# GDMCF/GDMCF

Hardware: AMD Instinct MI355X
Metric: training users/sec (higher is better)
Workload: dtype f32; 1 GPU; yelp-shape synthetic rows, batch=400/GPU, dims=[1000], T=5, noise_scale=0.01, linear-var, mean_type=x0, reweight, AdamW lr=1e-5 (BASELINE configs[1]); n_items=34395, global_batch=400, parallelism=dp1, batch_rows=device CSR rows (CsrBatch)

## Files before the change

gdmcf_amd/csrc/common.h:

```cpp
#pragma once
#include <hip/hip_runtime.h>
#include <stdint.h>
#include <stdio.h>

#include "../../include/gdmcf_hip.h"

typedef float f32x4 __attribute__((ext_vector_type(4)));
typedef f32x4 f32x4_u4 __attribute__((aligned(4)));

void gdmcf_set_error(const char* fmt, ...);

#define GD_CHECK_SHAPE(cond, msg)            \
    do {                                     \
        if (!(cond)) {                       \
            gdmcf_set_error("%s", msg);      \
            return GDMCF_E_SHAPE;            \
        }                                    \
    } while (0)

#define GD_CHECK_ARG(cond, msg)              \
    do {                                     \
        if (!(cond)) {                       \
            gdmcf_set_error("%s", msg);      \
            return GDMCF_E_ARG;              \
// ... 40 lines not shown
    return c;
}

struct GdShadow {
    void* p16;
    int64_t ld16;
    int64_t rows, cols;
};
bool gd_shadow_lookup(const void* f32, GdShadow* out);
int gd_cast_bf16(const float* src, int64_t ld, void* dst, int64_t ld16, int64_t rows, int64_t cols, hipStream_t s);

__device__ __forceinline__ unsigned short gd_bf16_bits(float x) {
    __bf16 h = (__bf16)x;
    return __builtin_bit_cast(unsigned short, h);
}

enum { GD_LAY_KC = 0, GD_LAY_MC = 1 };
enum { GD_EPI_SLAB = 0, GD_EPI_BIAS_ACT = 1, GD_EPI_LOSS = 2, GD_EPI_POST = 3, GD_EPI_STORE = 4, GD_EPI_ADAMW = 5 };

struct GdAdamHyper {
    float decay;
    float one_m_b1;
    float beta2;
    float one_m_b2;
    float bc2_sqrt;
    float eps;
    float neg_step;
    float grad_scale;
    float inv_bc2_sqrt;
    float pad_[3];
// ... 84 lines not shown
```

gdmcf_amd/csrc/linear.hip:

```cpp
#include <stdlib.h>

#include "common.h"

int gd_splitk_reduce(const float* slabs, int64_t slab_stride, int splits, int64_t ld_slab, int M, int N, int mode,
                     const float* bias, const float* rowscale, const float* aact, int64_t ldact, int act, float* out,
                     int64_t ldo, hipStream_t s);
int gd_colsum(const float* dZ, int64_t ld, const float* rs, int M, int N, float* db, hipStream_t s);
int gd_rowpart_reduce(const float* rowpart, int ld, int M, int nt, float* rowsum, hipStream_t s);

namespace {

static const int TARGET_WGS = getenv("GDMCF_TARGET_WGS") ? atoi(getenv("GDMCF_TARGET_WGS")) : 760;

thread_local int t_gemm_prec = GDMCF_GEMM_F32;

int pick_class(int M, int N, bool fused, int prec) {
    if (prec == GDMCF_GEMM_BF16 && M > 128) {
        const long pad = (long)gd_cdiv(M, 208) * 208;
        const long tiles = (pad / 208) * gd_cdiv(N, 256);
        const long rounds = (tiles + 255) / 256;
        if (pad * 10 <= (long)M * 11 && pad / 208 <= 2 && (!fused || tiles * 100 >= rounds * 256 * 85)) return 3;
    }
    if (prec == GDMCF_GEMM_F32X3 && M > 128 && N >= 128) {
        const long pad = (long)gd_cdiv(M, 208) * 208;
// ... 61 lines not shown
    g.bf16 = t_gemm_prec;
    g.A = e.dZ; g.lda = e.lddz; g.B = e.A; g.ldb = e.lda; g.M = N; g.N = K; g.K = M; g.splits = 1;
    g.m_fastest = gd_cdiv(N, gd_gemm_tile_m(cls)) <= gd_cdiv(K, gd_gemm_tile_n(cls));
    g.C = e.W; g.ldc = e.ldw; g.aux = e.exp_avg; g.aux2 = e.exp_avg_sq; g.prof_tag = 5;
    g.adam = gd_adam_hyper(e.lr, e.beta1, e.beta2, e.eps, e.weight_decay, e.step, e.grad_scale);
    g.adam_dev = t_gd_step_state ? &t_gd_step_state->hyper : nullptr;
    attach_result_shadow(g);
    attach_shadows(g, GD_LAY_MC, GD_LAY_MC);
    g.out2 = bias_col_request(e.a_scale_col, e.lda, e.rowscale, K, e.db);
    return GDMCF_OK;
}

int dw_adamw_finish(const GdDwAdamw& e, bool asked, const GdGemm& g, hipStream_t s) {
    if (asked && g.out2 == nullptr) return GDMCF_OK;
    if (e.db) return gd_colsum(e.dZ, e.lddz, e.rowscale, e.M, e.N, e.db, s);
    return GDMCF_OK;
}

}

extern "C" {

int gdmcf_gemm_precision(int mode) {
    const int prev = t_gemm_prec;
    if (mode == GDMCF_GEMM_F32 || mode == GDMCF_GEMM_BF16 || mode == GDMCF_GEMM_F32X3) t_gemm_prec = mode;
    return prev;
}

size_t gdmcf_linear_ws_bytes(int M, int N, int K) {
    if (M <= 0 || N <= 0 || K <= 0) return 0;
// ... 136 lines not shown
    GdGemm g = {};
    g.bf16 = t_gemm_prec;
    g.A = A; g.lda = lda; g.B = W; g.ldb = ldw; g.M = M; g.N = N; g.K = K; g.splits = 1;
    g.m_fastest = gd_cdiv(M, gd_gemm_tile_m(cls)) <= gd_cdiv(N, gd_gemm_tile_n(cls));
    g.bias = bias; g.aux = x_t; g.ldaux = ldxt; g.aux2 = z; g.ldaux2 = ldz;
    g.r0 = c1; g.r1 = c2; g.r2 = r1; g.r3 = r2; g.r4 = sigma;
    g.out2 = pred_out; g.ldout2 = ldp; g.C = x_next; g.ldc = ldxn; g.prof_tag = 3;
    attach_result_shadow(g);
    attach_shadows(g, GD_LAY_KC, GD_LAY_KC);
    return gd_gemm_launch(GD_LAY_KC, GD_LAY_KC, GD_EPI_POST, cls, g, s);
}

int gdmcf_linear_bwd_input_f32(const float* dZ, int64_t lddz, const float* W, int64_t ldw, const float* rowscale,
                               const float* Aact, int64_t ldact, int act, int M, int N, int K, float* dA,
                               int64_t ldda, void* ws, size_t ws_bytes, void* stream) {
    GD_CHECK_SHAPE(M > 0 && N > 0 && K > 0 && lddz >= N && ldw >= K && ldda >= K, "linear_bwd_input: bad shape");
    GD_CHECK_ARG(act == 0 || (act == 1 && Aact && ldact >= K), "linear_bwd_input: activation output missing");
    hipStream_t s = (hipStream_t)stream;
    const int cls = pick_class(M, K, false, t_gemm_prec);
    const int splits = pick_splits(M, K, N, cls, t_gemm_prec);
    const int64_t lds_ = round4(K);
    const size_t need = (size_t)splits * M * lds_ * sizeof(float);
    if (ws == nullptr || ws_bytes < need) {
        gdmcf_set_error("linear_bwd_input: workspace %zu < %zu bytes", ws_bytes, need);
        return GDMCF_E_WORKSPACE;
    }
    GdGemm g = {};
    g.bf16 = t_gemm_prec;
    g.A = dZ; g.lda = lddz; g.B = W; g.ldb = ldw; g.M = M; g.N = K; g.K = N;
    g.m_fastest = gd_cdiv(M, gd_gemm_tile_m(cls)) <= gd_cdiv(K, gd_gemm_tile_n(cls));
    g.splits = splits; g.C = (float*)ws; g.ldc = lds_; g.slab_stride = (int64_t)M * lds_; g.prof_tag = 4;
    g.ws_cap = ws_bytes;
    attach_shadows(g, GD_LAY_KC, GD_LAY_MC);
    int rc = gd_gemm_launch(GD_LAY_KC, GD_LAY_MC, GD_EPI_SLAB, cls, g, s);
    if (rc) return rc;
    const int real_splits = gd_cdiv(N, g.kchunk);
    return gd_splitk_reduce((const float*)ws, g.slab_stride, real_splits, lds_, M, K, 1, nullptr, rowscale, Aact,
                            ldact, act, dA, ldda, s);
}

int gdmcf_linear_bwd_weight_f32(const float* dZ, int64_t lddz, const float* A, int64_t lda, const float* rowscale,
                                int a_scale_col, int M, int N, int K, float* dW, int64_t lddw, float* db, int accumulate,
                                void* stream) {
    GD_CHECK_SHAPE(M > 0 && N > 0 && K > 0 && lddz >= N && lda >= K && lddw >= K, "linear_bwd_weight: bad shape");
    hipStream_t s = (hipStream_t)stream;
    const int cls = pick_class_dw(N, K, t_gemm_prec);
    GdGemm g = {};
    g.bf16 = t_gemm_prec;
    g.A = dZ; g.lda = lddz; g.B = A; g.ldb = lda; g.M = N; g.N = K; g.K = M; g.splits = 1;
    g.m_fastest = gd_cdiv(N, gd_gemm_tile_m(cls)) <= gd_cdiv(K, gd_gemm_tile_n(cls));
    g.C = dW; g.ldc = lddw; g.accumulate = accumulate; g.prof_tag = 5;
    attach_shadows(g, GD_LAY_MC, GD_LAY_MC);
    g.out2 = bias_col_request(a_scale_col, lda, rowscale, K, db);
// ... 60 lines not shown
```

gdmcf_amd/csrc/reduce.hip:

```cpp
#include "common.h"

namespace {

__global__ __launch_bounds__(256) void splitk_reduce_kernel(const float* __restrict__ slabs, int64_t slab_stride,
                                                            int splits, int64_t ld_slab, int M, int N, int mode,
                                                            const float* __restrict__ bias,
                                                            const float* __restrict__ rowscale,
                                                            const float* __restrict__ aact, int64_t ldact, int act,
                                                            float* __restrict__ out, int64_t ldo,
                                                            unsigned short* __restrict__ out16, int64_t ldo16, int vec) {
    const int m = blockIdx.y;
    const int n0 = (blockIdx.x * 256 + threadIdx.x) * 4;
    if (n0 >= N) return;
    float sv[4] = {0.f, 0.f, 0.f, 0.f};
    const float* p = slabs + (int64_t)m * ld_slab + n0;
    if (vec && n0 + 3 < N) {
        for (int k0 = 0; k0 < splits; k0 += 8) {
            f32x4 t[8];
#pragma unroll
            for (int u = 0; u < 8; ++u)
                t[u] = (k0 + u < splits) ? *reinterpret_cast<const f32x4*>(p + (int64_t)(k0 + u) * slab_stride)
                                         : f32x4{0.f, 0.f, 0.f, 0.f};
#pragma unroll
            for (int u = 0; u < 8; ++u)
                if (k0 + u < splits) { sv[0] += t[u].x; sv[1] += t[u].y; sv[2] += t[u].z; sv[3] += t[u].w; }
        }
    } else {
// ... 7 lines not shown
        const int n = n0 + j;
        if (n >= N) break;
        float s = sv[j];
        if (mode == 0) {
            if (bias) s += bias[n];
            if (act == 1) s = tanhf(s);
        } else {
            if (rowscale) s *= rs;
            if (act == 1) {
                const float h = aact[(int64_t)m * ldact + n];
                s *= (1.f - h * h);
            }
        }
        out[(int64_t)m * ldo + n] = s;
        if (out16) out16[(int64_t)m * ldo16 + n] = gd_bf16_bits(s);
    }
}

__global__ __launch_bounds__(256) void rowscale_kernel(const float* __restrict__ A, int64_t lda,
                                                       const float* __restrict__ rs, int M, int K,
                                                       float* __restrict__ out, int64_t ldo,
                                                       unsigned short* __restrict__ out16, int64_t ldo16, int bias_col) {
    const int m = blockIdx.y, k = (blockIdx.x * 256 + threadIdx.x) * 4;
    if (bias_col && blockIdx.x == 0 && threadIdx.x == 0) out[(int64_t)m * ldo + K] = rs[m];
    if (k >= K) return;
    const float r = rs[m];
    const float* a = A + (int64_t)m * lda + k;
    float* o = out + (int64_t)m * ldo + k;
    float v[4];
    if (k + 3 < K) {
        const f32x4 t = *reinterpret_cast<const f32x4_u4*>(a);
        v[0] = t.x * r; v[1] = t.y * r; v[2] = t.z * r; v[3] = t.w * r;
        *reinterpret_cast<f32x4_u4*>(o) = f32x4{v[0], v[1], v[2], v[3]};
    } else {
        for (int j = 0; j < 4; ++j)
            if (k + j < K) o[j] = v[j] = a[j] * r;
    }
    if (out16)
        for (int j = 0; j < 4; ++j)
            if (k + j < K) out16[(int64_t)m * ldo16 + k + j] = gd_bf16_bits(v[j]);
}

__global__ __launch_bounds__(256) void colsum_kernel(const float* __restrict__ dZ, int64_t ld,
                                                     const float* __restrict__ rs, int M, int N,
                                                     float* __restrict__ db) {
    __shared__ float part[4][64];
    const int lane = threadIdx.x & 63, wave = threadIdx.x >> 6;
    const int n = blockIdx.x * 64 + lane;
    const int nc = min(n, N - 1);
    float s = 0.f;
    int m = wave;
    for (; m + 28 < M; m += 32) {
        float v[8];
#pragma unroll
        for (int j = 0; j < 8; ++j) v[j] = dZ[(int64_t)(m + 4 * j) * ld + nc] * (rs ? rs[m + 4 * j] : 1.f);
#pragma unroll
        for (int j = 0; j < 8; ++j) s += v[j];
// ... 58 lines not shown

}

int gd_splitk_reduce(const float* slabs, int64_t slab_stride, int splits, int64_t ld_slab, int M, int N, int mode,
                     const float* bias, const float* rowscale, const float* aact, int64_t ldact, int act, float* out,
                     int64_t ldo, hipStream_t s) {
    GdShadow sh;
    const bool has16 = gd_shadow_lookup(out, &sh) && sh.rows == M && sh.cols == N;
    const int vec = (ld_slab % 4 == 0) && (slab_stride % 4 == 0) && gd_aligned16(slabs);
    hipLaunchKernelGGL(splitk_reduce_kernel, dim3(gd_cdiv(N, 1024), M), dim3(256), 0, s, slabs, slab_stride,
                       splits, ld_slab, M, N, mode, bias, rowscale, aact, ldact, act, out, ldo,
                       has16 ? (unsigned short*)sh.p16 : nullptr, has16 ? sh.ld16 : 0, vec);
    return gd_launch_status("splitk_reduce");
}

int gd_colsum(const float* dZ, int64_t ld, const float* rs, int M, int N, float* db, hipStream_t s) {
    hipLaunchKernelGGL(colsum_kernel, dim3(gd_cdiv(N, 64)), dim3(256), 0, s, dZ, ld, rs, M, N, db);
    return gd_launch_status("colsum");
}

int gd_rowpart_reduce(const float* rowpart, int ld, int M, int nt, float* rowsum, hipStream_t s) {
    hipLaunchKernelGGL(rowpart_reduce_kernel, dim3(gd_cdiv(M, 4)), dim3(256), 0, s, rowpart, ld, M, nt, rowsum);
    return gd_launch_status("rowpart_reduce");
}

int gd_cast_bf16(const float* src, int64_t ld, void* dst, int64_t ld16, int64_t rows, int64_t cols, hipStream_t s) {
    const int64_t total = rows * ((cols + 7) / 8);
    const int64_t blocks = (total + 255) / 256;
    hipLaunchKernelGGL(cast_bf16_kernel, dim3((unsigned)(blocks < 16384 ? blocks : 16384)), dim3(256), 0, s, src, ld,
                       (unsigned short*)dst, ld16, rows, cols);
// ... 3 lines not shown
```

gdmcf_amd/csrc/rows.hip:

```cpp
#include "common.h"

namespace {

__device__ __forceinline__ float block_sum_256(float v, float* red) {
#pragma unroll
    for (int o = 32; o > 0; o >>= 1) v += __shfl_down(v, o, 64);
    __syncthreads();
    if ((threadIdx.x & 63) == 0) red[threadIdx.x >> 6] = v;
    __syncthreads();
    return red[0] + red[1] + red[2] + red[3];
}

__global__ __launch_bounds__(256) void row_norms_kernel(const float* __restrict__ X, int64_t ld, int cols,
                                                       float* __restrict__ norm, float* __restrict__ inv_norm) {
    __shared__ float red[4];
    const float* x = X + (int64_t)blockIdx.x * ld;
    float ss = 0.f;
    const int c4 = cols & ~3;
    for (int c = threadIdx.x * 4; c < c4; c += 1024) {
        const f32x4 t = *reinterpret_cast<const f32x4_u4*>(x + c);
        ss += t.x * t.x + t.y * t.y + t.z * t.z + t.w * t.w;
    }
    if (threadIdx.x < cols - c4) ss += x[c4 + threadIdx.x] * x[c4 + threadIdx.x];
    const float n = sqrtf(block_sum_256(ss, red));
// ... 155 lines not shown
}

__global__ __launch_bounds__(256) void emb_gather_w_kernel(const float* __restrict__ W1, int64_t ldw, int I, int E, int N,
                                                           float* __restrict__ W1e) {
    const int idx = blockIdx.x * 256 + threadIdx.x;
    if (idx < N * E) W1e[idx] = W1[(int64_t)(idx / E) * ldw + I + (idx % E)];
}

__global__ __launch_bounds__(256) void emb_bwd_demb_kernel(const float* __restrict__ dZ1, int64_t lddz,
                                                           const float* __restrict__ W1e, int E, int N,
                                                           float* __restrict__ demb) {
    const int m = blockIdx.x;
    const int lane = threadIdx.x & 63, wave = threadIdx.x >> 6;
    for (int e = wave; e < E; e += 4) {
        float s = 0.f;
        for (int n = lane; n < N; n += 64) s += dZ1[(int64_t)m * lddz + n] * W1e[(int64_t)n * E + e];
        for (int o = 32; o > 0; o >>= 1) s += __shfl_xor(s, o);
        if (lane == 0) demb[(int64_t)m * E + e] = s;
    }
}

__global__ __launch_bounds__(64) void emb_bwd_w_kernel(const float* __restrict__ demb, const float* __restrict__ temb,
                                                       int M, int E, float* __restrict__ dWe,
                                                       float* __restrict__ dbe) {
    const int idx = blockIdx.x, lane = threadIdx.x;
    float s = 0.f;
    if (idx < E * E) {
        const int e = idx / E, f = idx % E;
        for (int m = lane; m < M; m += 64) s += demb[(int64_t)m * E + e] * temb[(int64_t)m * E + f];
    } else {
        const int e = idx - E * E;
// ... 24 lines not shown
    const int64_t u = row_ids ? row_ids[b] : b;
    for (int64_t j = indptr[u] + threadIdx.x; j < indptr[u + 1]; j += 256) {
        const int c = indices[j];
        if (c >= 0 && c < I) row[c] = values ? values[j] : 1.f;
    }
}

__global__ __launch_bounds__(256) void scale_kernel(const float* __restrict__ a, int64_t n, float s,
                                                    float* __restrict__ out) {
    const int64_t i = (int64_t)blockIdx.x * 256 + threadIdx.x;
    if (i < n) out[i] = a[i] * s;
}

}

extern "C" {

int gdmcf_row_norms_f32(const float* X, int64_t ld, int rows, int cols, float* norm, float* inv_norm, void* stream) {
    GD_CHECK_SHAPE(rows > 0 && cols > 0 && ld >= cols, "row_norms: bad shape");
    GD_CHECK_ARG(X && (norm || inv_norm), "row_norms: null pointer");
    hipLaunchKernelGGL(row_norms_kernel, dim3(rows), dim3(256), 0, (hipStream_t)stream, X, ld, cols, norm, inv_norm);
    return gd_launch_status("row_norms");
}

int gdmcf_normalize_rows_bwd_f32(const float* dY, int64_t lddy, const float* Y, int64_t ldy, const float* inv_norm, int rows,
                                 int cols, float* dX, int64_t lddx, void* stream) {
    GD_CHECK_SHAPE(rows > 0 && cols > 0 && lddy >= cols && ldy >= cols && lddx >= cols, "normalize_rows_bwd: bad shape");
    GD_CHECK_ARG(dY && Y && inv_norm && dX, "normalize_rows_bwd: null pointer");
    hipLaunchKernelGGL(normalize_rows_bwd_kernel<false>, dim3(rows), dim3(256), 0, (hipStream_t)stream, dY, lddy, Y, ldy,
                       inv_norm, cols, dX, lddx, nullptr, nullptr, GdAdamHyper{}, nullptr);
// ... 46 lines not shown
    GD_CHECK_SHAPE(n >= 0 && rows > 0 && cols > 0 && ldw >= cols && (n == 0 || lds >= cols), "scatter_rows_adamw: bad shape");
    GD_CHECK_ARG(W && exp_avg && exp_avg_sq && (n == 0 || (src && index)) && step >= 1, "scatter_rows_adamw: null pointer");
    const GdAdamHyper h = gd_adam_hyper(lr, beta1, beta2, eps, weight_decay, step, grad_scale);
    {
        GdProfScope prof(6, 24.0 * (double)rows * cols, (hipStream_t)stream);
        hipLaunchKernelGGL(scatter_rows_adamw_kernel, dim3(gd_cdiv(rows, SCATTER_ADAM_ROWS)), dim3(256), 0, (hipStream_t)stream,
                           src, lds, index, n, rows, cols, W, ldw, exp_avg, exp_avg_sq, h, t_gd_step_state);
    }
    return gd_launch_status("scatter_rows_adamw");
}

int gdmcf_emb_bwd_f32(const float* dZ1, int64_t lddz, const float* W1, int64_t ldw, int I, int E, const float* temb,
                      int M, int N, float* demb_ws, float* dWe, float* dbe, void* stream) {
    GD_CHECK_SHAPE(M > 0 && N > 0 && E > 0 && ldw >= I + E && lddz >= N, "emb_bwd: bad shape");
    hipStream_t s = (hipStream_t)stream;
    float* W1e = demb_ws + (size_t)M * E;
    hipLaunchKernelGGL(emb_gather_w_kernel, dim3(gd_cdiv(N * E, 256)), dim3(256), 0, s, W1, ldw, I, E, N, W1e);
    hipLaunchKernelGGL(emb_bwd_demb_kernel, dim3(M), dim3(256), 0, s, dZ1, lddz, W1e, E, N, demb_ws);
    hipLaunchKernelGGL(emb_bwd_w_kernel, dim3(E * E + E), dim3(64), 0, s, demb_ws, temb, M, E, dWe, dbe);
    return gd_launch_status("emb_bwd");
}

int gdmcf_densify_rows_f32(const int64_t* indptr, const int32_t* indices, const float* values, const int64_t* row_ids,
                           int B, int I, float* out, int64_t ldo, void* stream) {
    GD_CHECK_SHAPE(B > 0 && I > 0 && ldo >= I, "densify_rows: bad shape");
    hipLaunchKernelGGL(densify_rows_kernel, dim3(B), dim3(256), 0, (hipStream_t)stream, indptr, indices, values, row_ids,
                       I, out, ldo);
    return gd_launch_status("densify_rows");
}

int gdmcf_scale_f32(const float* acc, int64_t n, float scale, float* out, void* stream) {
    GD_CHECK_SHAPE(n > 0, "scale: empty");
    hipLaunchKernelGGL(scale_kernel, dim3((unsigned)((n + 255) / 256)), dim3(256), 0, (hipStream_t)stream, acc, n,
                       scale, out);
    return gd_launch_status("scale");
// ... 4 lines not shown
```

gdmcf_amd/engine.py:

```python

import ctypes
import os

import torch

from . import _lib
from . import engine_core as core
from .engine_core import EngineBase, _Bufs, _ceil64, with_precision


class DenoiserEngine(EngineBase):
    def __init__(self, model):
        super().__init__(model)
        self._wshadow = {}
        self.input_grad_first = False
        self.weight_waiters = {}
        self.static_grads = False
        self._grad_bufs = {}
        self._gemm_side = os.environ.get("GDMCF_GEMM_SIDE", "0") == "1"
        self._side2 = None
        self._side2_used = False
        self._wt_on = os.environ.get("GDMCF_FWD_WT", "1") == "1"

    def _grad_like(self, p):
# ... 198 lines not shown
        if g.stride(-1) != 1:
            g = g.contiguous()
        return self._backward(sv, g, None)

    def _backward(self, sv, dz_last, rowscale):
        lib, st = self.lib, _lib.stream_ptr()
        bufs, layers, B = sv["bufs"], sv["layers"], sv["B"]
        m = self.model
        L = len(layers)
        grads_w = [None] * L
        grads_b = [None] * L
        dWe = dbe = None
        fused = self.fused_opt if self.grad_sink is None else None
        dz, rs = dz_last, rowscale
        dw_queue = [] if (fused is not None and self.gemm_dtype == "f32" and os.environ.get("GDMCF_DW_MULTI", "1") != "0") else None

        def input_grad(li, w, A_prev):
            nonlocal dWe, dbe
            N, K = w.shape
            if li > 0:
                dprev = bufs.dzs[li - 1]
                self._input_grad(bufs, B, w, N, K, dz, rs, A_prev, layers[li - 1][2], dprev, st)
                return dprev
            dWe = self._grad_like(m.emb_layer.weight)
            dbe = self._grad_like(m.emb_layer.bias)
            core.emb_bwd(lib, bufs, dz, w, self.I, self.E, B, N, dWe, dbe, st)
            return None

        def weight_grad(li, w, bias, A_prev):
            db = self._grad_like(bias)
            scol = int(rs is None and li == 0 and getattr(bufs, "xin_ones", False) and A_prev.stride(0) > w.shape[1])
            A_use, scol = self._row_scaled(bufs, B, w.shape[1], A_prev, rs, scol, st)
            fs = fused.fused_state(w) if fused is not None else None
            dW = self._grad_like(w) if fs is None else None
            if fs is None and self._gemm_side and self.grad_sink is None and li == L - 1 and L > 1:
                if self._side2 is None:
                    self._side2 = torch.cuda.Stream()
                self._side2.wait_stream(torch.cuda.current_stream())
                with torch.cuda.stream(self._side2):
                    self._weight_grad(bufs, B, w, dz, rs, A_use, scol, dW, db, None, _lib.stream_ptr())
                self._side2_used = True
            else:
                self._weight_grad(bufs, B, w, dz, rs, A_use, scol, dW, db, fs, st, queue=dw_queue)
            grads_w[li], grads_b[li] = dW, db
            if self.grad_sink is not None:
                self.grad_sink(w, dW)
                self.grad_sink(bias, db)
                grads_w[li] = grads_b[li] = None

        for li in range(L - 1, -1, -1):
            w, bias, _ = layers[li]
            A_prev = bufs.acts[li - 1] if li > 0 else bufs.xin
            if fused is not None or self.input_grad_first:
                nxt = input_grad(li, w, A_prev)
                weight_grad(li, w, bias, A_prev)
            else:
                weight_grad(li, w, bias, A_prev)
                nxt = input_grad(li, w, A_prev)
            dz, rs = nxt, None
        if dw_queue:
            arr = (_lib.GdDwAdamw * len(dw_queue))(*[e for e, _ in dw_queue])
            _lib.check(lib.gdmcf_linear_bwd_weight_adamw_multi_f32(ctypes.addressof(arr), len(dw_queue), st))
            for _, w in dw_queue:
                torch.autograd.graph.increment_version(w)
        if self._side2_used:
            torch.cuda.current_stream().wait_stream(self._side2)
            self._side2_used = False
        if self.grad_sink is not None:
# ... 153 lines not shown
```

gdmcf_amd/engine_core.py:

```python
import functools

import torch

from . import _lib


def _ceil64(n):
    return (int(n) + 63) // 64 * 64


class _Bufs:
    pass


_GEMM_MODES = {k: _lib.CONSTANTS["GDMCF_GEMM_" + k.upper()] for k in ("f32", "bf16", "f32x3")}


def with_precision(fn):
    @functools.wraps(fn)
    def wrapped(self, *a, **kw):
        prev = self.lib.gdmcf_gemm_precision(_GEMM_MODES[self.gemm_dtype])
        try:
            return fn(self, *a, **kw)
        finally:
# ... 105 lines not shown
    _lib.check(lib.gdmcf_gather_fwd_f32(
        p, ldp, _lib.ptr(base), c.indptr.data_ptr() if c is not None else None, c.indices.data_ptr() if c is not None else None,
        batch.row_ids.data_ptr() if c is not None else None, tb, ldt, I, ap, lda, te, ldte, E, _lib.ptr(bias), act, B, N, o, ldo, st))


def latent_step(lib, A, M, v, p_cur, c1, c2, e, act, B, N, K, p_next, h_next, st):
    (a, lda), (m, ldm), (pc, ldpc), (pn, ldpn), (h, ldh) = _pl(A), _pl(M), _pl(p_cur), _pl(p_next), _pl(h_next)
    _lib.check(lib.gdmcf_latent_step_f32(a, lda, m, ldm, _lib.ptr(v), pc, ldpc, c1.data_ptr(), c2.data_ptr(), _lib.ptr(e), act,
                                         B, N, K, pn, ldpn, h, ldh, None, 0, st))


def linear_bwd_input(lib, bufs, dz, W, rs, A_prev, act_prev, B, N, K, d_prev, st):
    (z, ldz), (w, ldw), (a, lda), (d, ldd) = _pl(dz), _pl(W), _pl(A_prev), _pl(d_prev)
    _lib.check(lib.gdmcf_linear_bwd_input_f32(z, ldz, w, ldw, _lib.ptr(rs), a, lda, act_prev, B, N, K, d, ldd,
                                              bufs.ws.data_ptr(), bufs.ws_bytes, st))


def linear_bwd_weight(lib, dz, A, rs, scol, B, N, K, dW, db, st):
    (z, ldz), (a, lda) = _pl(dz), _pl(A)
    _lib.check(lib.gdmcf_linear_bwd_weight_f32(z, ldz, a, lda, _lib.ptr(rs), scol, B, N, K, dW.data_ptr(), dW.stride(0),
                                               _lib.ptr(db), 0, st))


def adamw_args(fs, w):
    if fs["exp_avg"].stride() != w.stride() or fs["exp_avg_sq"].stride() != w.stride():
        raise RuntimeError("gdmcf_amd: the moments of a fused weight must share its leading dimension")
    return (fs["exp_avg"].data_ptr(), fs["exp_avg_sq"].data_ptr(), fs["lr"], fs["beta1"], fs["beta2"], fs["eps"],
            fs["weight_decay"], fs["step"], fs["grad_scale"])


# ... 199 lines not shown
        _lib.check(self.lib.gdmcf_eps_target_f32(
            noise.data_ptr(), noise.stride(0), bufs.xt.data_ptr(), bufs.xt.stride(0), x0.data_ptr(), x0.stride(0), ts.data_ptr(),
            spec["r1_0"].data_ptr(), spec["r2_0"].data_ptr(), int(bool(spec.get("t0_likelihood", True))), B, self.I,
            target.data_ptr(), target.stride(0), alpha.data_ptr(), rowdiv.data_ptr(), _lib.stream_ptr()))
        return target, alpha, rowdiv

    def _rowscale_of(self, bufs, gloss):
        if isinstance(gloss, float):
            return bufs.gradcoef * gloss
        return (gloss.to(torch.float32) * bufs.gradcoef).contiguous()

    def _fused_state(self, w):
        fused = self.fused_opt if self.grad_sink is None else None
        return fused.fused_state(w) if fused is not None else None

    def _row_scaled(self, bufs, B, K, A, rs, scol, st):
        if rs is None:
            return A, scol
        rowscale(self.lib, A, rs, B, K, bufs.hs, st)
        return bufs.hs, int(bufs.hs.stride(0) > K)

    def _weight_grad(self, bufs, B, w, dz, rs, A, scol, dW, db, fs, st, queue=None):
        N, K = w.shape
        if fs is None:
            linear_bwd_weight(self.lib, dz, A, rs, scol, B, N, K, dW, db, st)
            return
        args = dw_adamw_args(dz, A, rs, scol, B, N, K, w, db, fs)
        if queue is not None:
            queue.append((_lib.GdDwAdamw(*args), w))
            return
        linear_bwd_weight_adamw(self.lib, args, st)
        if not (self.gemm_dtype == "bf16" and _lib.shadow_info(w.data_ptr()) is not None):
            torch.autograd.graph.increment_version(w)

# ... 3 lines not shown
```

include/gdmcf_hip.h:

```cpp
#ifndef GDMCF_HIP_H
#define GDMCF_HIP_H
#include <stddef.h>
#include <stdint.h>

#ifdef __cplusplus
extern "C" {
#endif

#define GDMCF_OK 0
#define GDMCF_E_SHAPE (-1)
#define GDMCF_E_ARG (-2)
#define GDMCF_E_UNSUPPORTED (-3)
#define GDMCF_E_HIP (-4)
#define GDMCF_E_WORKSPACE (-5)

int gdmcf_version(void);
const char* gdmcf_last_error(void);
int gdmcf_device_info(int* n_cu, int* wave_size, char* arch_host, int arch_len);
int gdmcf_debug_last_gemm(void);

int gdmcf_prof_enable(int on);
int gdmcf_prof_collect(int cap, int* tags_host, float* ms_host, double* work_host);

#define GDMCF_N_TABLES 13
// ... 71 lines not shown
                              void* stream);
int gdmcf_linear_loss_fwd_bits_f32(const float* A, int64_t lda, const float* W, int64_t ldw, const float* bias,
                                   const uint32_t* target_bits, int64_t ldbits, const float* alpha, int M, int N, int K,
                                   float* out, int64_t ldo, float* diff, int64_t ldd, float* rowpart, float* rowsum,
                                   void* stream);
int gdmcf_linear_posterior_fwd_f32(const float* A, int64_t lda, const float* W, int64_t ldw,
                                   const float* bias, const float* x_t, int64_t ldxt,
                                   const float* c1, const float* c2, const float* r1,
                                   const float* r2, const float* sigma, const float* z,
                                   int64_t ldz, int M, int N, int K, float* x_next,
                                   int64_t ldxn, float* pred_out, int64_t ldp, void* stream);
int gdmcf_linear_bwd_input_f32(const float* dZ, int64_t lddz, const float* W, int64_t ldw,
                               const float* rowscale, const float* Aact, int64_t ldact, int act,
                               int M, int N, int K, float* dA, int64_t ldda, void* ws,
                               size_t ws_bytes, void* stream);
int gdmcf_linear_bwd_weight_f32(const float* dZ, int64_t lddz, const float* A, int64_t lda,
                                const float* rowscale, int a_scale_col, int M, int N, int K,
                                float* dW, int64_t lddw, float* db, int accumulate, void* stream);
int gdmcf_linear_bwd_weight_adamw_f32(const float* dZ, int64_t lddz, const float* A, int64_t lda,
                                      const float* rowscale, int a_scale_col, int M, int N, int K, float* W,
                                      int64_t ldw, float* exp_avg, float* exp_avg_sq, float* db, float lr,
                                      float beta1, float beta2, float eps, float weight_decay, int step,
                                      float grad_scale, void* stream);
typedef struct GdDwAdamw {
    const float* dZ;
    int64_t lddz;
    const float* A;
    int64_t lda;
    const float* rowscale;
    int a_scale_col, M, N, K;
// ... 144 lines not shown
```

Baseline: 312,900 users/s.

## Fuse split-K reduce with rowscale and embedding-grad demb into one backward glue kernel

Adds a combined backward glue kernel that performs the split-K reduction of the input gradient and, in the same launch, computes the rowscaled activations for the weight gradient and the embedding dL/demb dot products from the reduced row held in shared memory. The engine reorders backward to input-grad-first when glue is enabled, so the separate rowscale and emb_bwd_demb launches and the re-read of dA are skipped. This cuts kernel launches and global memory round trips. In exchange the glue blocks do extra per-row work, the W1e reads are strided, and block imbalance may appear.

```diff
diff --git a/gdmcf_amd/csrc/common.h b/gdmcf_amd/csrc/common.h
--- a/gdmcf_amd/csrc/common.h
+++ b/gdmcf_amd/csrc/common.h
@@ -78,6 +78,12 @@
     __bf16 h = (__bf16)x;
     return __builtin_bit_cast(unsigned short, h);
 }
+
+__device__ __forceinline__ float gd_emb_acc(float s, float dz, float w) { return __builtin_fmaf(dz, w, s); }
+
+void gd_emb_gather_w(const float* W1, int64_t ldw, int I, int E, int M, int N, float* demb_ws, hipStream_t s);
+void gd_emb_bwd_demb(const float* dZ1, int64_t lddz, int E, int M, int N, float* demb_ws, hipStream_t s);
+int gd_emb_bwd_w(const float* demb, const float* temb, int M, int E, float* dWe, float* dbe, hipStream_t s);
 
 enum { GD_LAY_KC = 0, GD_LAY_MC = 1 };
 enum { GD_EPI_SLAB = 0, GD_EPI_BIAS_ACT = 1, GD_EPI_LOSS = 2, GD_EPI_POST = 3, GD_EPI_STORE = 4, GD_EPI_ADAMW = 5 };
diff --git a/gdmcf_amd/csrc/linear.hip b/gdmcf_amd/csrc/linear.hip
--- a/gdmcf_amd/csrc/linear.hip
+++ b/gdmcf_amd/csrc/linear.hip
@@ -5,6 +5,11 @@
 int gd_splitk_reduce(const float* slabs, int64_t slab_stride, int splits, int64_t ld_slab, int M, int N, int mode,
                      const float* bias, const float* rowscale, const float* aact, int64_t ldact, int act, float* out,
                      int64_t ldo, hipStream_t s);
+bool gd_glue_takes_emb(int N);
+int gd_bwd_glue(const float* slabs, int64_t slab_stride, int splits, int64_t ld_slab, int M, int N, const float* rowscale,
+                const float* aact, int64_t ldact, int act, float* out, int64_t ldo, const float* A_scale, int64_t lda_scale,
+                const float* rs_scale, int K_scale, float* out_scale, int64_t ldo_scale, const float* W1e, int E, float* demb,
+                hipStream_t s);
 int gd_colsum(const float* dZ, int64_t ld, const float* rs, int M, int N, float* db, hipStream_t s);
 int gd_rowpart_reduce(const float* rowpart, int ld, int M, int nt, float* rowsum, hipStream_t s);
 
@@ -99,6 +104,38 @@
 int dw_adamw_finish(const GdDwAdamw& e, bool asked, const GdGemm& g, hipStream_t s) {
     if (asked && g.out2 == nullptr) return GDMCF_OK;
     if (e.db) return gd_colsum(e.dZ, e.lddz, e.rowscale, e.M, e.N, e.db, s);
+    return GDMCF_OK;
+}
+
+int bwd_input_product(const char* who, const float* dZ, int64_t lddz, const float* W, int64_t ldw, const float* Aact, int64_t ldact,
+                      int act, int M, int N, int K, int64_t ldda, void* ws, size_t ws_bytes, hipStream_t s, int& real_splits,
+                      int64_t& lds_) {
+    if (!(M > 0 && N > 0 && K > 0 && lddz >= N && ldw >= K && ldda >= K)) {
+        gdmcf_set_error("%s: bad shape", who);
+        return GDMCF_E_SHAPE;
+    }
+    if (!(act == 0 || (act == 1 && Aact && ldact >= K))) {
+        gdmcf_set_error("%s: activation output missing", who);
+        return GDMCF_E_ARG;
+    }
+    const int cls = pick_class(M, K, false, t_gemm_prec);
+    const int splits = pick_splits(M, K, N, cls, t_gemm_prec);
+    lds_ = round4(K);
+    const size_t need = (size_t)splits * M * lds_ * sizeof(float);
+    if (ws == nullptr || ws_bytes < need) {
+        gdmcf_set_error("%s: workspace %zu < %zu bytes", who, ws_bytes, need);
+        return GDMCF_E_WORKSPACE;
+    }
+    GdGemm g = {};
+    g.bf16 = t_gemm_prec;
+    g.A = dZ; g.lda = lddz; g.B = W; g.ldb = ldw; g.M = M; g.N = K; g.K = N;
+    g.m_fastest = gd_cdiv(M, gd_gemm_tile_m(cls)) <= gd_cdiv(K, gd_gemm_tile_n(cls));
+    g.splits = splits; g.C = (float*)ws; g.ldc = lds_; g.slab_stride = (int64_t)M * lds_; g.prof_tag = 4;
+    g.ws_cap = ws_bytes;
+    attach_shadows(g, GD_LAY_KC, GD_LAY_MC);
+    int rc = gd_gemm_launch(GD_LAY_KC, GD_LAY_MC, GD_EPI_SLAB, cls, g, s);
+    if (rc) return rc;
+    real_splits = gd_cdiv(N, g.kchunk);
     return GDMCF_OK;
 }
 
@@ -265,29 +302,43 @@
 int gdmcf_linear_bwd_input_f32(const float* dZ, int64_t lddz, const float* W, int64_t ldw, const float* rowscale,
                                const float* Aact, int64_t ldact, int act, int M, int N, int K, float* dA,
                                int64_t ldda, void* ws, size_t ws_bytes, void* stream) {
-    GD_CHECK_SHAPE(M > 0 && N > 0 && K > 0 && lddz >= N && ldw >= K && ldda >= K, "linear_bwd_input: bad shape");
-    GD_CHECK_ARG(act == 0 || (act == 1 && Aact && ldact >= K), "linear_bwd_input: activation output missing");
-    hipStream_t s = (hipStream_t)stream;
-    const int cls = pick_class(M, K, false, t_gemm_prec);
-    const int splits = pick_splits(M, K, N, cls, t_gemm_prec);
-    const int64_t lds_ = round4(K);
-    const size_t need = (size_t)splits * M * lds_ * sizeof(float);
-    if (ws == nullptr || ws_bytes < need) {
-        gdmcf_set_error("linear_bwd_input: workspace %zu < %zu bytes", ws_bytes, need);
-        return GDMCF_E_WORKSPACE;
-    }
-    GdGemm g = {};
-    g.bf16 = t_gemm_prec;
-    g.A = dZ; g.lda = lddz; g.B = W; g.ldb = ldw; g.M = M; g.N = K; g.K = N;
-    g.m_fastest = gd_cdiv(M, gd_gemm_tile_m(cls)) <= gd_cdiv(K, gd_gemm_tile_n(cls));
-    g.splits = splits; g.C = (float*)ws; g.ldc = lds_; g.slab_stride = (int64_t)M * lds_; g.prof_tag = 4;
-    g.ws_cap = ws_bytes;
-    attach_shadows(g, GD_LAY_KC, GD_LAY_MC);
-    int rc = gd_gemm_launch(GD_LAY_KC, GD_LAY_MC, GD_EPI_SLAB, cls, g, s);
-    if (rc) return rc;
-    const int real_splits = gd_cdiv(N, g.kchunk);
-    return gd_splitk_reduce((const float*)ws, g.slab_stride, real_splits, lds_, M, K, 1, nullptr, rowscale, Aact,
+    hipStream_t s = (hipStream_t)stream;
+    int real_splits;
+    int64_t lds_;
+    int rc = bwd_input_product("linear_bwd_input", dZ, lddz, W, ldw, Aact, ldact, act, M, N, K, ldda, ws, ws_bytes, s, real_splits, lds_);
+    if (rc) return rc;
+    return gd_splitk_reduce((const float*)ws, (int64_t)M * lds_, real_splits, lds_, M, K, 1, nullptr, rowscale, Aact,
                             ldact, act, dA, ldda, s);
+}
+
+int gdmcf_linear_bwd_input_glue_f32(const float* dZ, int64_t lddz, const float* W, int64_t ldw, const float* rowscale,
+                                    const float* Aact, int64_t ldact, int act, int M, int N, int K, float* dA, int64_t ldda,
+                                    void* ws, size_t ws_bytes, const float* A_scale, int64_t lda_scale, const float* rs_scale,
+                                    int K_scale, float* out_scale, int64_t ldo_scale, const float* W_first, int64_t ldw_first,
+                                    int I_cols, int E, float* demb_ws, const float* temb, float* dWe, float* dbe, void* stream) {
+    const bool scale = A_scale || rs_scale || out_scale || K_scale > 0;
+    GD_CHECK_ARG(!scale || (A_scale && rs_scale && out_scale), "linear_bwd_input_glue: incomplete scale group");
+    GD_CHECK_SHAPE(!scale || (K_scale > 0 && lda_scale >= K_scale && ldo_scale >= K_scale), "linear_bwd_input_glue: bad scale shape");
+    const bool emb = W_first != nullptr && E > 0;
+    GD_CHECK_ARG(!emb || (demb_ws && temb && dWe && dbe), "linear_bwd_input_glue: incomplete embedding group");
+    GD_CHECK_SHAPE(!emb || (I_cols >= 0 && ldw_first >= (int64_t)I_cols + E), "linear_bwd_input_glue: bad embedding shape");
+    hipStream_t s = (hipStream_t)stream;
+    const bool fuse_emb = emb && gd_glue_takes_emb(K);
+    if (fuse_emb) gd_emb_gather_w(W_first, ldw_first, I_cols, E, M, K, demb_ws, s);
+    int real_splits;
+    int64_t lds_;
+    int rc = bwd_input_product("linear_bwd_input_glue", dZ, lddz, W, ldw, Aact, ldact, act, M, N, K, ldda, ws, ws_bytes, s, real_splits,
+                               lds_);
+    if (rc) return rc;
+    rc = gd_bwd_glue((const float*)ws, (int64_t)M * lds_, real_splits, lds_, M, K, rowscale, Aact, ldact, act, dA, ldda,
+                     scale ? A_scale : nullptr, lda_scale, rs_scale, K_scale, out_scale, ldo_scale,
+                     fuse_emb ? demb_ws + (size_t)M * E : nullptr, E, demb_ws, s);
+    if (rc || !emb) return rc;
+    if (!fuse_emb) {
+        gd_emb_gather_w(W_first, ldw_first, I_cols, E, M, K, demb_ws, s);
+        gd_emb_bwd_demb(dA, ldda, E, M, K, demb_ws, s);
+    }
+    return gd_emb_bwd_w(demb_ws, temb, M, E, dWe, dbe, s);
 }
 
 int gdmcf_linear_bwd_weight_f32(const float* dZ, int64_t lddz, const float* A, int64_t lda, const float* rowscale,
diff --git a/gdmcf_amd/csrc/reduce.hip b/gdmcf_amd/csrc/reduce.hip
--- a/gdmcf_amd/csrc/reduce.hip
+++ b/gdmcf_amd/csrc/reduce.hip
@@ -2,15 +2,12 @@
 
 namespace {
 
-__global__ __launch_bounds__(256) void splitk_reduce_kernel(const float* __restrict__ slabs, int64_t slab_stride,
-                                                            int splits, int64_t ld_slab, int M, int N, int mode,
-                                                            const float* __restrict__ bias,
-                                                            const float* __restrict__ rowscale,
-                                                            const float* __restrict__ aact, int64_t ldact, int act,
-                                                            float* __restrict__ out, int64_t ldo,
-                                                            unsigned short* __restrict__ out16, int64_t ldo16, int vec) {
-    const int m = blockIdx.y;
-    const int n0 = (blockIdx.x * 256 + threadIdx.x) * 4;
+__device__ __forceinline__ void splitk_reduce_body(int bx, int m, const float* __restrict__ slabs, int64_t slab_stride, int splits,
+                                                   int64_t ld_slab, int N, int mode, const float* __restrict__ bias,
+                                                   const float* __restrict__ rowscale, const float* __restrict__ aact, int64_t ldact,
+                                                   int act, float* __restrict__ out, int64_t ldo, unsigned short* __restrict__ out16,
+                                                   int64_t ldo16, int vec, float* row) {
+    const int n0 = (bx * 256 + threadIdx.x) * 4;
     if (n0 >= N) return;
     float sv[4] = {0.f, 0.f, 0.f, 0.f};
     const float* p = slabs + (int64_t)m * ld_slab + n0;
@@ -48,15 +45,26 @@
         }
         out[(int64_t)m * ldo + n] = s;
         if (out16) out16[(int64_t)m * ldo16 + n] = gd_bf16_bits(s);
-    }
-}
-
-__global__ __launch_bounds__(256) void rowscale_kernel(const float* __restrict__ A, int64_t lda,
-                                                       const float* __restrict__ rs, int M, int K,
-                                                       float* __restrict__ out, int64_t ldo,
-                                                       unsigned short* __restrict__ out16, int64_t ldo16, int bias_col) {
-    const int m = blockIdx.y, k = (blockIdx.x * 256 + threadIdx.x) * 4;
-    if (bias_col && blockIdx.x == 0 && threadIdx.x == 0) out[(int64_t)m * ldo + K] = rs[m];
+        if (row) row[n] = s;
+    }
+}
+
+__global__ __launch_bounds__(256) void splitk_reduce_kernel(const float* __restrict__ slabs, int64_t slab_stride,
+                                                            int splits, int64_t ld_slab, int M, int N, int mode,
+                                                            const float* __restrict__ bias,
+                                                            const float* __restrict__ rowscale,
+                                                            const float* __restrict__ aact, int64_t ldact, int act,
+                                                            float* __restrict__ out, int64_t ldo,
+                                                            unsigned short* __restrict__ out16, int64_t ldo16, int vec) {
+    splitk_reduce_body(blockIdx.x, blockIdx.y, slabs, slab_stride, splits, ld_slab, N, mode, bias, rowscale, aact, ldact, act, out,
+                       ldo, out16, ldo16, vec, nullptr);
+}
+
+__device__ __forceinline__ void rowscale_body(int bx, int m, const float* __restrict__ A, int64_t lda, const float* __restrict__ rs,
+                                              int K, float* __restrict__ out, int64_t ldo, unsigned short* __restrict__ out16,
+                                              int64_t ldo16, int bias_col) {
+    const int k = (bx * 256 + threadIdx.x) * 4;
+    if (bias_col && bx == 0 && threadIdx.x == 0) out[(int64_t)m * ldo + K] = rs[m];
     if (k >= K) return;
     const float r = rs[m];
     const float* a = A + (int64_t)m * lda + k;
@@ -75,6 +83,51 @@
             if (k + j < K) out16[(int64_t)m * ldo16 + k + j] = gd_bf16_bits(v[j]);
 }
 
+__global__ __launch_bounds__(256) void rowscale_kernel(const float* __restrict__ A, int64_t lda,
+                                                       const float* __restrict__ rs, int M, int K,
+                                                       float* __restrict__ out, int64_t ldo,
+                                                       unsigned short* __restrict__ out16, int64_t ldo16, int bias_col) {
+    rowscale_body(blockIdx.x, blockIdx.y, A, lda, rs, K, out, ldo, out16, ldo16, bias_col);
+}
+
+struct GdGlue {
+    const float* slabs; int64_t slab_stride; int splits; int64_t ld_slab; int N;
+    const float* rowscale; const float* aact; int64_t ldact; int act;
+    float* out; int64_t ldo; unsigned short* out16; int64_t ldo16; int vec;
+    int bx_r;
+    const float* W1e; int E; float* demb;
+    const float* A; int64_t lda; const float* rs; int K; float* hs; int64_t ldhs; unsigned short* hs16; int64_t ldhs16; int bias_col;
+};
+constexpr int GLUE_ROW = 1024;
+
+__global__ __launch_bounds__(256) void bwd_glue_kernel(GdGlue a) {
+    __shared__ float row[GLUE_ROW];
+    const int m = blockIdx.y;
+    if ((int)blockIdx.x >= a.bx_r) {
+        rowscale_body(blockIdx.x - a.bx_r, m, a.A, a.lda, a.rs, a.K, a.hs, a.ldhs, a.hs16, a.ldhs16, a.bias_col);
+        return;
+    }
+    splitk_reduce_body(blockIdx.x, m, a.slabs, a.slab_stride, a.splits, a.ld_slab, a.N, 1, nullptr, a.rowscale, a.aact, a.ldact, a.act,
+                       a.out, a.ldo, a.out16, a.ldo16, a.vec, a.W1e ? row : nullptr);
+    if (a.W1e == nullptr) return;
+    __syncthreads();
+    const int lane = threadIdx.x & 63, wave = threadIdx.x >> 6;
+    for (int e = wave; e < a.E; e += 4) {
+        float wv[GLUE_ROW / 64];
+#pragma unroll
+        for (int u = 0; u < GLUE_ROW / 64; ++u) wv[u] = a.W1e[(int64_t)min(lane + 64 * u, a.N - 1) * a.E + e];
+        float s = 0.f;
+#pragma unroll
+        for (int u = 0; u < GLUE_ROW / 64; ++u) {
+            const int n = lane + 64 * u;
+            const float t = gd_emb_acc(s, row[min(n, a.N - 1)], wv[u]);
+            s = n < a.N ? t : s;
+        }
+        for (int o = 32; o > 0; o >>= 1) s += __shfl_xor(s, o);
+        if (lane == 0) a.demb[(int64_t)m * a.E + e] = s;
+    }
+}
+
 __global__ __launch_bounds__(256) void colsum_kernel(const float* __restrict__ dZ, int64_t ld,
                                                      const float* __restrict__ rs, int M, int N,
                                                      float* __restrict__ db) {
@@ -163,6 +216,39 @@
     return gd_launch_status("splitk_reduce");
 }
 
+bool gd_glue_takes_emb(int N) { return N <= GLUE_ROW; }
+
+int gd_bwd_glue(const float* slabs, int64_t slab_stride, int splits, int64_t ld_slab, int M, int N, const float* rowscale,
+                const float* aact, int64_t ldact, int act, float* out, int64_t ldo, const float* A_scale, int64_t lda_scale,
+                const float* rs_scale, int K_scale, float* out_scale, int64_t ldo_scale, const float* W1e, int E, float* demb,
+                hipStream_t s) {
+    GdShadow sh;
+    GdGlue a = {};
+    const bool has16 = gd_shadow_lookup(out, &sh) && sh.rows == M && sh.cols == N;
+    a.slabs = slabs; a.slab_stride = slab_stride; a.splits = splits; a.ld_slab = ld_slab; a.N = N;
+    a.rowscale = rowscale; a.aact = aact; a.ldact = ldact; a.act = act;
+    a.out = out; a.ldo = ldo; a.out16 = has16 ? (unsigned short*)sh.p16 : nullptr; a.ldo16 = has16 ? sh.ld16 : 0;
+    a.vec = (ld_slab % 4 == 0) && (slab_stride % 4 == 0) && gd_aligned16(slabs);
+    a.bx_r = gd_cdiv(N, 1024);
+    if (W1e) {
+        if (!gd_glue_takes_emb(N)) {
+            gdmcf_set_error("bwd_glue: embedding part on rows of more than %d columns", GLUE_ROW);
+            return GDMCF_E_UNSUPPORTED;
+        }
+        a.W1e = W1e; a.E = E; a.demb = demb;
+    }
+    int bx_s = 0;
+    if (A_scale) {
+        const bool hs16 = gd_shadow_lookup(out_scale, &sh) && sh.rows == M && sh.cols == K_scale;
+        a.A = A_scale; a.lda = lda_scale; a.rs = rs_scale; a.K = K_scale; a.hs = out_scale; a.ldhs = ldo_scale;
+        a.hs16 = hs16 ? (unsigned short*)sh.p16 : nullptr; a.ldhs16 = hs16 ? sh.ld16 : 0;
+        a.bias_col = ldo_scale > K_scale;
+        bx_s = gd_cdiv(K_scale, 1024);
+    }
+    hipLaunchKernelGGL(bwd_glue_kernel, dim3(a.bx_r + bx_s, M), dim3(256), 0, s, a);
+    return gd_launch_status("bwd_glue");
+}
+
 int gd_colsum(const float* dZ, int64_t ld, const float* rs, int M, int N, float* db, hipStream_t s) {
     hipLaunchKernelGGL(colsum_kernel, dim3(gd_cdiv(N, 64)), dim3(256), 0, s, dZ, ld, rs, M, N, db);
     return gd_launch_status("colsum");
diff --git a/gdmcf_amd/csrc/rows.hip b/gdmcf_amd/csrc/rows.hip
--- a/gdmcf_amd/csrc/rows.hip
+++ b/gdmcf_amd/csrc/rows.hip
@@ -193,7 +193,7 @@
     const int lane = threadIdx.x & 63, wave = threadIdx.x >> 6;
     for (int e = wave; e < E; e += 4) {
         float s = 0.f;
-        for (int n = lane; n < N; n += 64) s += dZ1[(int64_t)m * lddz + n] * W1e[(int64_t)n * E + e];
+        for (int n = lane; n < N; n += 64) s = gd_emb_acc(s, dZ1[(int64_t)m * lddz + n], W1e[(int64_t)n * E + e]);
         for (int o = 32; o > 0; o >>= 1) s += __shfl_xor(s, o);
         if (lane == 0) demb[(int64_t)m * E + e] = s;
     }
@@ -248,6 +248,19 @@
 
 }
 
+void gd_emb_gather_w(const float* W1, int64_t ldw, int I, int E, int M, int N, float* demb_ws, hipStream_t s) {
+    hipLaunchKernelGGL(emb_gather_w_kernel, dim3(gd_cdiv(N * E, 256)), dim3(256), 0, s, W1, ldw, I, E, N, demb_ws + (size_t)M * E);
+}
+
+void gd_emb_bwd_demb(const float* dZ1, int64_t lddz, int E, int M, int N, float* demb_ws, hipStream_t s) {
+    hipLaunchKernelGGL(emb_bwd_demb_kernel, dim3(M), dim3(256), 0, s, dZ1, lddz, demb_ws + (size_t)M * E, E, N, demb_ws);
+}
+
+int gd_emb_bwd_w(const float* demb, const float* temb, int M, int E, float* dWe, float* dbe, hipStream_t s) {
+    hipLaunchKernelGGL(emb_bwd_w_kernel, dim3(E * E + E), dim3(64), 0, s, demb, temb, M, E, dWe, dbe);
+    return gd_launch_status("emb_bwd");
+}
+
 extern "C" {
 
 int gdmcf_row_norms_f32(const float* X, int64_t ld, int rows, int cols, float* norm, float* inv_norm, void* stream) {
@@ -324,11 +337,9 @@
                       int M, int N, float* demb_ws, float* dWe, float* dbe, void* stream) {
     GD_CHECK_SHAPE(M > 0 && N > 0 && E > 0 && ldw >= I + E && lddz >= N, "emb_bwd: bad shape");
     hipStream_t s = (hipStream_t)stream;
-    float* W1e = demb_ws + (size_t)M * E;
-    hipLaunchKernelGGL(emb_gather_w_kernel, dim3(gd_cdiv(N * E, 256)), dim3(256), 0, s, W1, ldw, I, E, N, W1e);
-    hipLaunchKernelGGL(emb_bwd_demb_kernel, dim3(M), dim3(256), 0, s, dZ1, lddz, W1e, E, N, demb_ws);
-    hipLaunchKernelGGL(emb_bwd_w_kernel, dim3(E * E + E), dim3(64), 0, s, demb_ws, temb, M, E, dWe, dbe);
-    return gd_launch_status("emb_bwd");
+    gd_emb_gather_w(W1, ldw, I, E, M, N, demb_ws, s);
+    gd_emb_bwd_demb(dZ1, lddz, E, M, N, demb_ws, s);
+    return gd_emb_bwd_w(demb_ws, temb, M, E, dWe, dbe, s);
 }
 
 int gdmcf_densify_rows_f32(const int64_t* indptr, const int32_t* indices, const float* values, const int64_t* row_ids,
diff --git a/gdmcf_amd/engine.py b/gdmcf_amd/engine.py
--- a/gdmcf_amd/engine.py
+++ b/gdmcf_amd/engine.py
@@ -236,14 +236,31 @@
         fused = self.fused_opt if self.grad_sink is None else None
         dz, rs = dz_last, rowscale
         dw_queue = [] if (fused is not None and self.gemm_dtype == "f32" and os.environ.get("GDMCF_DW_MULTI", "1") != "0") else None
+        glue = L > 1 and os.environ.get("GDMCF_BWD_GLUE", "1") != "0"
+        input_first = fused is not None or self.input_grad_first or (glue and self.grad_sink is None and not self._gemm_side)
+        glue = glue and input_first
+        done = dict(hs=False, emb=False)
 
         def input_grad(li, w, A_prev):
             nonlocal dWe, dbe
             N, K = w.shape
             if li > 0:
                 dprev = bufs.dzs[li - 1]
-                self._input_grad(bufs, B, w, N, K, dz, rs, A_prev, layers[li - 1][2], dprev, st)
+                scale = emb = None
+                if glue and li == L - 1 and rs is not None:
+                    scale = (A_prev, rs, K, bufs.hs)
+                if glue and li == 1 and self.E > 0:
+                    dWe = self._grad_like(m.emb_layer.weight)
+                    dbe = self._grad_like(m.emb_layer.bias)
+                    emb = (layers[0][0], self.I, self.E, dWe, dbe)
+                if scale is None and emb is None:
+                    self._input_grad(bufs, B, w, N, K, dz, rs, A_prev, layers[li - 1][2], dprev, st)
+                    return dprev
+                core.linear_bwd_input_glue(lib, bufs, dz, w, rs, A_prev, layers[li - 1][2], B, N, K, dprev, scale, emb, st)
+                done["hs"], done["emb"] = done["hs"] or scale is not None, done["emb"] or emb is not None
                 return dprev
+            if done["emb"]:
+                return None
             dWe = self._grad_like(m.emb_layer.weight)
             dbe = self._grad_like(m.emb_layer.bias)
             core.emb_bwd(lib, bufs, dz, w, self.I, self.E, B, N, dWe, dbe, st)
@@ -252,7 +269,7 @@
         def weight_grad(li, w, bias, A_prev):
             db = self._grad_like(bias)
             scol = int(rs is None and li == 0 and getattr(bufs, "xin_ones", False) and A_prev.stride(0) > w.shape[1])
-            A_use, scol = self._row_scaled(bufs, B, w.shape[1], A_prev, rs, scol, st)
+            A_use, scol = self._row_scaled(bufs, B, w.shape[1], A_prev, rs, scol, st, written=done["hs"] and li == L - 1)
             fs = fused.fused_state(w) if fused is not None else None
             dW = self._grad_like(w) if fs is None else None
             if fs is None and self._gemm_side and self.grad_sink is None and li == L - 1 and L > 1:
@@ -273,7 +290,7 @@
         for li in range(L - 1, -1, -1):
             w, bias, _ = layers[li]
             A_prev = bufs.acts[li - 1] if li > 0 else bufs.xin
-            if fused is not None or self.input_grad_first:
+            if input_first:
                 nxt = input_grad(li, w, A_prev)
                 weight_grad(li, w, bias, A_prev)
             else:
diff --git a/gdmcf_amd/engine_core.py b/gdmcf_amd/engine_core.py
--- a/gdmcf_amd/engine_core.py
+++ b/gdmcf_amd/engine_core.py
@@ -143,6 +143,20 @@
     (z, ldz), (w, ldw), (a, lda), (d, ldd) = _pl(dz), _pl(W), _pl(A_prev), _pl(d_prev)
     _lib.check(lib.gdmcf_linear_bwd_input_f32(z, ldz, w, ldw, _lib.ptr(rs), a, lda, act_prev, B, N, K, d, ldd,
                                               bufs.ws.data_ptr(), bufs.ws_bytes, st))
+
+
+def linear_bwd_input_glue(lib, bufs, dz, W, rs, A_prev, act_prev, B, N, K, d_prev, scale, emb, st):
+    (z, ldz), (w, ldw), (a, lda), (d, ldd) = _pl(dz), _pl(W), _pl(A_prev), _pl(d_prev)
+    sc = (None, 0, None, 0, None, 0)
+    if scale is not None:
+        (sa, slda), (so, sldo) = _pl(scale[0]), _pl(scale[3])
+        sc = (sa, slda, scale[1].data_ptr(), scale[2], so, sldo)
+    em = (None, 0, 0, 0, None, None, None, None)
+    if emb is not None:
+        wf, ldwf = _pl(emb[0])
+        em = (wf, ldwf, emb[1], emb[2], bufs.demb.data_ptr(), bufs.temb.data_ptr(), emb[3].data_ptr(), emb[4].data_ptr())
+    _lib.check(lib.gdmcf_linear_bwd_input_glue_f32(z, ldz, w, ldw, _lib.ptr(rs), a, lda, act_prev, B, N, K, d, ldd,
+                                                   bufs.ws.data_ptr(), bufs.ws_bytes, *sc, *em, st))
 
 
 def linear_bwd_weight(lib, dz, A, rs, scol, B, N, K, dW, db, st):
@@ -372,10 +386,11 @@
         fused = self.fused_opt if self.grad_sink is None else None
         return fused.fused_state(w) if fused is not None else None
 
-    def _row_scaled(self, bufs, B, K, A, rs, scol, st):
+    def _row_scaled(self, bufs, B, K, A, rs, scol, st, written=False):
         if rs is None:
             return A, scol
-        rowscale(self.lib, A, rs, B, K, bufs.hs, st)
+        if not written:
+            rowscale(self.lib, A, rs, B, K, bufs.hs, st)
         return bufs.hs, int(bufs.hs.stride(0) > K)
 
     def _weight_grad(self, bufs, B, w, dz, rs, A, scol, dW, db, fs, st, queue=None):
diff --git a/include/gdmcf_hip.h b/include/gdmcf_hip.h
--- a/include/gdmcf_hip.h
+++ b/include/gdmcf_hip.h
@@ -109,6 +109,13 @@
                                const float* rowscale, const float* Aact, int64_t ldact, int act,
                                int M, int N, int K, float* dA, int64_t ldda, void* ws,
                                size_t ws_bytes, void* stream);
+int gdmcf_linear_bwd_input_glue_f32(const float* dZ, int64_t lddz, const float* W, int64_t ldw,
+                                    const float* rowscale, const float* Aact, int64_t ldact, int act, int M,
+                                    int N, int K, float* dA, int64_t ldda, void* ws, size_t ws_bytes,
+                                    const float* A_scale, int64_t lda_scale, const float* rs_scale, int K_scale,
+                                    float* out_scale, int64_t ldo_scale, const float* W_first, int64_t ldw_first,
+                                    int I_cols, int E, float* demb_ws, const float* temb, float* dWe, float* dbe,
+                                    void* stream);
 int gdmcf_linear_bwd_weight_f32(const float* dZ, int64_t lddz, const float* A, int64_t lda,
                                 const float* rowscale, int a_scale_col, int M, int N, int K,
                                 float* dW, int64_t lddw, float* db, int accumulate, void* stream);
```

Measured after the change: 313,300 users/s (median of 6 runs). No clear change (+0.1%).
